# rampasek/DrVAE

Hardware: AMD Instinct MI355X
Metric: DrVAE ELBO training samples/sec (batch x L) (higher is better)
Workload: dtype f32; 1 GPU; cfg2: DrVAE bortezomib shape: 978 genes, z1=z3=100, enc-z1 800, dec-x 600, enc-z3/dec-z1 200, batch 150/GPU, L=2; global_batch=150, L=2, parallelism=dp1, launch=hipGraph replay, feed=resident, side_chain_cus=64, rccl_ranks=0, params=2321758

## Files before the change

### drvae_amd/csrc/gemm.hip

```cpp
#include "gemm_common.inc"

namespace {

#include "gemm_pipe.inc"


struct Operand {
    const float* base;
    int64_t ld;
    int n_line, n_pos;
};

__device__ __forceinline__ float4 ld_fast(const Operand& o, int line, int pos, int vec) {
    const float* p = o.base + (int64_t)line * o.ld + pos;
    if (vec == 4) return *reinterpret_cast<const float4*>(p);
    if (vec == 2) {
        const float2 a = *reinterpret_cast<const float2*>(p), b = *reinterpret_cast<const float2*>(p + 2);
        return make_float4(a.x, a.y, b.x, b.y);
    }
    return make_float4(p[0], p[1], p[2], p[3]);
}

__device__ __forceinline__ float4 ld_edge(const Operand& o, int line, int pos) {
    const bool lok = line < o.n_line;
    const float* row = o.base + (int64_t)(lok ? line : o.n_line - 1) * o.ld;
    float e[4];
#pragma unroll
    for (int j = 0; j < 4; ++j) {
        const int q = pos + j;
        const float v = row[q < o.n_pos ? q : o.n_pos - 1];
        e[j] = (lok && q < o.n_pos) ? v : 0.f;
    }
    return make_float4(e[0], e[1], e[2], e[3]);
}

template <int BM, int RPT>
__device__ __forceinline__ int heads_row0(int grp) { return (grp & 1) * (BM / 2) + (grp >> 1) * RPT; }

template <int BM, int BN, int KS, int NT>
__device__ __forceinline__ void heads_epilogue(const dv_gemm_desc& g, const dv_heads_epi& he, const float* red, int m0,
                                               int tn, int tiles_n, int pre_s0, int pre_s1) {
    constexpr int HB = BN / 2, RPT = BM / (NT / HB);
    constexpr bool PRE = (KS == 8 && BN == 32);
    static_assert(!PRE || RPT == 1, "prefetched bounds: one row per thread");
    static_assert((HB == 32 || HB == 16) && RPT >= 1, "half tile = 16 or 32 adjacent lanes");
    static_assert((NT / HB) % 2 == 0 && (BM / 2) % RPT == 0, "row groups come in pairs");
    const int tid = threadIdx.x, c = tid % HB, r0 = heads_row0<BM, RPT>(tid / HB);
    const int col0 = tn * HB + c, col1 = g.split + col0;
    const bool ok = col0 < g.split && col1 < g.N;
    const int cc0 = ok ? col0 : g.split - 1, cc1 = ok ? col1 : g.N - 1;
    float sc0 = 1.f, sc1 = 1.f, bi0 = 0.f, bi1 = 0.f;
    if (g.scale) {
        sc0 = g.scale[cc0];
        sc1 = g.scale[cc1];
    }
    if (g.bias) {
        bi0 = g.bias[cc0];
        bi1 = g.bias[cc1];
    }
    const bool use_res = g.resid != nullptr && col0 < g.resid_cols;
#pragma unroll
    for (int e = 0; e < RPT; ++e) {
        const int row = m0 + r0 + e;
        const bool rok = row < g.M;
        const int rc = rok ? row : g.M - 1;
        float v0 = 0.f, v1 = 0.f;
#pragma unroll
        for (int w = 0; w < KS; ++w) {
            v0 += red[(w * BM + r0 + e) * (BN + 1) + c];
            v1 += red[(w * BM + r0 + e) * (BN + 1) + HB + c];
        }
        float a0 = dv_act(g.act0, v0 * g.alpha * sc0 + bi0) + g.shift0;
        if (use_res) a0 += g.resid[(int64_t)rc * g.ldr + cc0];
        if (he.mode == DV_HEADS_NLL && g.act1 == DV_ACT_SOFTPLUS) {
            const float pre = v1 * g.alpha * sc1 + bi1;
            const float e_ = __expf(-fabsf(pre));
            const float r1 = __frcp_rn(1.f + e_);
            const float sd = fmaxf(pre, 0.f) + dv_log1p_hw(e_, r1) + g.shift1;
            const float sig = (pre >= 0.f ? 1.f : e_) * r1;
            const float is = __frcp_rn(sd);
            const float xv = he.x[(int64_t)(he.xidx ? he.xidx[rc] : rc) * he.ldx + cc0];
            const float cf = he.coef[rc];
            const float t = (xv - a0) * is;
            float acc = ok ? kLog2PiG + 2.f * __logf(sd) + t * t : 0.f;
            if (ok && rok) {
                g.C[(int64_t)row * g.ldc + col0] = cf * t * is;
                g.C[(int64_t)row * g.ldc + col1] = cf * (t * t - 1.f) * is * sig;
            }
#pragma unroll
            for (int off = HB / 2; off > 0; off >>= 1) acc += __shfl_xor(acc, off, 64);
            if (c == 0 && rok) he.part[(int64_t)row * tiles_n + tn] = -0.5f * acc;
            continue;
        }
        const float a1 = dv_act(g.act1, v1 * g.alpha * sc1 + bi1) + g.shift1;
        if (he.mode == DV_HEADS_SAMPLE) {
            if (ok && rok) {
                g.C[(int64_t)row * g.ldc + col0] = a0;
                g.C[(int64_t)row * g.ldc + col1] = a1;
                if (row < he.n_src) {
                    const float std_ = expf(0.5f * a1);
                    const int s0 = he.seg_ptr ? (PRE ? pre_s0 : he.seg_ptr[row]) : row;
                    const int s1 = he.seg_ptr ? (PRE ? pre_s1 : he.seg_ptr[row + 1]) : row + 1;
                    for (int t = s0; t < s1; ++t) {
                        const int64_t s = he.seg_rows ? he.seg_rows[t] : t;
                        const float z = he.eps[s * he.lde + col0] * std_ + a0;
                        he.out[s * he.ldo + col0] = z;
                        if (he.out2) he.out2[s * he.ldo2 + col0] = z - he.sub[s * he.lds + col0];
                        if (he.out3) {
                            const int t3 = he.out3_idx[s];
                            if (t3 >= 0) he.out3[(int64_t)t3 * he.ldo3 + col0] = z;
                        }
                        if (he.out4)
                            for (int u = he.out4_ptr[s]; u < he.out4_ptr[s + 1]; ++u) he.out4[(int64_t)u * he.ldo4 + col0] = z;
                    }
                }
            }
        } else {
            const float xv = he.x[(int64_t)(he.xidx ? he.xidx[rc] : rc) * he.ldx + cc0];
            const float cf = he.coef[rc];
            const float d = xv - a0, v = a1 * a1;
            float acc = ok ? kLog2PiG + logf(v) + d * d / v : 0.f;
            float gm = d / v, gs = -1.f / a1 + d * d / (v * a1);
            if (g.act1 != DV_ACT_IDENTITY) gs *= dv_dact_from_y(g.act1, a1 - g.shift1);
            gm *= cf;
            gs *= cf;
            if (ok && rok) {
                g.C[(int64_t)row * g.ldc + col0] = gm;
                g.C[(int64_t)row * g.ldc + col1] = gs;
            }
#pragma unroll
            for (int off = HB / 2; off > 0; off >>= 1) acc += __shfl_xor(acc, off, 64);
            if (c == 0 && rok) he.part[(int64_t)row * tiles_n + tn] = -0.5f * acc;
        }
    }
}

template <int BM, int BN, int BK, int KS, bool AKC, bool BKC, int PS = 0>
constexpr int gemm_smem_floats() {
    if constexpr (PS > 0) return PipeGeom<BM, BN, BK, BM / 32, BN / 32, KS, PS, AKC, BKC>::SMEM_FL;
    constexpr int stage = (AKC ? BM : BK) * ((AKC ? BK : BM) + 4) + (BKC ? BN : BK) * ((BKC ? BK : BN) + 4);
    constexpr int red = (KS > 1) ? KS * BM * (BN + 1) : 0;
    return 2 * stage > red ? 2 * stage : red;
}

template <int BM, int BN, int BK, int WM, int WN, int KS, bool AKC, bool BKC, bool PAIR = false, bool MI16 = false, int PS = 0>
__device__ __forceinline__ void gemm_body(const dv_gemm_desc& g, const LoadCfg& lc, float* smem, int bid, int nwg,
                                          const dv_heads_epi* he = nullptr) {
    static_assert(!PAIR || (AKC && BKC && KS > 1 && WM == 1 && WN == 1), "paired heads: forward layout, K-split tiling");
    constexpr int HB = BN / 2;
    static_assert(!MI16 || (KS == 1 && !PAIR), "16x16x4 tiles: unsplit K only");
    constexpr int TS = MI16 ? 16 : 32;
    constexpr int AR = MI16 ? 4 : 16;
// ... 82 lines not shown
        for (int p = 0; p < B_NP; ++p) {
            const int l = b_l + p * B_LPP;
            rb[p] = ld_edge(ob, BKC ? (PAIR ? bline(l) : n0 + l) : (k0 + l), BKC ? (k0 + b_c * 4) : (n0 + b_c * 4));
        }
    };
    auto stage_store = [&](float* buf, const float4 (&ra)[A_NP], const float4 (&rb)[B_NP]) {
        float* sA = buf;
        float* sB = buf + A_ELEMS;
#pragma unroll
        for (int p = 0; p < A_NP; ++p) {
            *reinterpret_cast<float4*>(&sA[(a_l + p * A_LPP) * LDA_S + a_c * 4]) = ra[p];
        }
#pragma unroll
        for (int p = 0; p < B_NP; ++p) {
            float4 v = rb[p];
            if (BM < 128 && !AKC && !BKC) {
                v.x = oc == 0 ? 1.f : v.x;
                v.y = oc == 1 ? 1.f : v.y;
                v.z = oc == 2 ? 1.f : v.z;
                v.w = oc == 3 ? 1.f : v.w;
            }
            *reinterpret_cast<float4*>(&sB[(b_l + p * B_LPP) * LDB_S + b_c * 4]) = v;
        }
    };

    typename std::conditional<MI16, f32x4, f32x16>::type acc[TM][TN];
#pragma unroll
    for (int i = 0; i < TM; ++i)
#pragma unroll
        for (int j = 0; j < TN; ++j)
#pragma unroll
            for (int r = 0; r < AR; ++r) acc[i][j][r] = 0.f;

    int pre_s0 = 0, pre_s1 = 0;
    if constexpr (PAIR && KS == 8 && BN == 32) {
        if (he->mode == DV_HEADS_SAMPLE && he->seg_ptr != nullptr) {
            const int prow = m0 + heads_row0<BM, 1>(tid / (BN / 2));
            if (prow < he->n_src && prow < g.M) {
                pre_s0 = he->seg_ptr[prow];
                pre_s1 = he->seg_ptr[prow + 1];
            }
        }
    }
    const int kb = ks_id * KW + lh * KH;
    auto read_frags = [&](const float* sA, float (&fa)[TM][KH], float (&fb)[TN][KH]) {
        const float* sB = sA + A_ELEMS;
#pragma unroll
        for (int i = 0; i < TM; ++i) {
            const int row = wm * TM * TS + i * TS + li;
#pragma unroll
            for (int s = 0; s < KH; s += 4) {
                if (AKC) {
                    const float4 v = *reinterpret_cast<const float4*>(&sA[row * LDA_S + kb + s]);
                    fa[i][s] = v.x;
                    fa[i][s + 1] = v.y;
                    fa[i][s + 2] = v.z;
                    fa[i][s + 3] = v.w;
                } else {
#pragma unroll
                    for (int e = 0; e < 4; ++e) fa[i][s + e] = sA[(kb + s + e) * LDA_S + row];
                }
            }
        }
#pragma unroll
        for (int j = 0; j < TN; ++j) {
            const int col = wn * TN * TS + j * TS + li;
#pragma unroll
            for (int s = 0; s < KH; s += 4) {
                if (BKC) {
                    const float4 v = *reinterpret_cast<const float4*>(&sB[col * LDB_S + kb + s]);
                    fb[j][s] = v.x;
                    fb[j][s + 1] = v.y;
                    fb[j][s + 2] = v.z;
                    fb[j][s + 3] = v.w;
                } else {
#pragma unroll
                    for (int e = 0; e < 4; ++e) fb[j][s + e] = sB[(kb + s + e) * LDB_S + col];
                }
            }
        }
    };
    auto mma = [&](const float (&fa)[TM][KH], const float (&fb)[TN][KH]) {
#pragma unroll
        for (int s = 0; s < KH; ++s)
#pragma unroll
            for (int i = 0; i < TM; ++i)
#pragma unroll
                for (int j = 0; j < TN; ++j) {
                    if constexpr (MI16)
                        acc[i][j] = __builtin_amdgcn_mfma_f32_16x16x4f32(fa[i][s], fb[j][s], acc[i][j], 0, 0, 0);
                    else if (DV_DBG & 2)
                        acc[i][j][s & 15] += fa[i][s] * fb[j][s];
                    else
                        acc[i][j] = __builtin_amdgcn_mfma_f32_32x32x2f32(fa[i][s], fb[j][s], acc[i][j], 0, 0, 0);
                }
    };
    auto compute = [&](const float* sA) {
        float fa[TM][KH], fb[TN][KH];
        read_frags(sA, fa, fb);
        mma(fa, fb);
    };

    const int nkt = (g.K + BK - 1) / BK, nfull = g.K / BK;
    float* const buf0 = smem;
    float* const buf1 = smem + STAGE;
    if constexpr (PS > 0) {
        if (!(DV_DBG & 64))
            pipe_loop<BM, BN, BK, WM, WN, KS, PS, AKC, BKC, (BM < 128 && !AKC && !BKC)>(
                g, smem, m0, n0, [&](int l) { return m0 + l < g.M ? m0 + l : g.M - 1; }, bline, acc);
        if (DV_DBG & 128) {
            if (acc[0][0][0] == 12345.678f) g.C[0] = acc[0][0][1];
            return;
        }
        __syncthreads();
    } else if (wg_fast && nfull >= 1) {
        const float* pa[A_NP];
        const float* pb[B_NP];
#pragma unroll
        for (int p = 0; p < A_NP; ++p) {
            const int l = a_l + p * A_LPP;
            int line = AKC ? (m0 + l) : l;
            if (AKC) line = line < g.M ? line : g.M - 1;
            pa[p] = g.A + (int64_t)line * g.lda + (AKC ? a_c * 4 : (m0 + a_c * 4 < g.M ? m0 + a_c * 4 : 0));
        }
#pragma unroll
        for (int p = 0; p < B_NP; ++p) {
            const int l = b_l + p * B_LPP;
            const int line = BKC ? bline(l) : l;
            pb[p] = g.B + (int64_t)line * g.ldb + (BKC ? b_c * 4 : (n0 + b_c * 4 < g.N ? n0 + b_c * 4 : 0));
        }
        const int64_t step_a = AKC ? (int64_t)BK : (int64_t)BK * g.lda;
        const int64_t step_b = BKC ? (int64_t)BK : (int64_t)BK * g.ldb;
        const int va = lc.vecA, vb = lc.vecB;
        auto ldv = [](const float* p, int vec) -> float4 {
            if (vec == 4) return *reinterpret_cast<const float4*>(p);
            if (vec == 2) {
                const float2 a = *reinterpret_cast<const float2*>(p), b = *reinterpret_cast<const float2*>(p + 2);
                return make_float4(a.x, a.y, b.x, b.y);
            }
            return make_float4(p[0], p[1], p[2], p[3]);
        };
        auto ldv_tail = [](const float* p, int vec, int left) -> float4 {
// ... 119 lines not shown
    if constexpr (MI16) {
#pragma unroll
        for (int i = 0; i < TM; ++i)
#pragma unroll
            for (int j = 0; j < TN; ++j) {
                float a4[4];
#pragma unroll
                for (int r = 0; r < 4; ++r) a4[r] = acc[i][j][r];
                const int rbase = m0 + wm * TM * TS + i * TS + 4 * lh;
                epi_store_col<4, (BM < 128)>(g, a4, n0 + wn * TN * TS + j * TS + li, [rbase](int r) { return rbase + r; });
            }
    } else if constexpr (KS == 1) {
#pragma unroll
        for (int i = 0; i < TM; ++i)
#pragma unroll
            for (int j = 0; j < TN; ++j) {
                float a16[16];
#pragma unroll
                for (int r = 0; r < 16; ++r) a16[r] = acc[i][j][r];
                const int rbase = m0 + wm * TM * 32 + i * 32 + 4 * lh;
                epi_store_col<16, (BM < 128)>(g, a16, n0 + wn * TN * 32 + j * 32 + li,
                                  [rbase](int r) { return rbase + (r & 3) + 8 * (r >> 2); });
            }
    } else {
        float* red = smem;
        if constexpr (PAIR) {
#pragma unroll
            for (int j = 0; j < TN; ++j)
#pragma unroll
                for (int r = 0; r < 16; ++r) {
                    const int row = (r & 3) + 8 * (r >> 2) + 4 * lh;
                    red[(ks_id * BM + row) * (BN + 1) + j * 32 + li] = acc[0][j][r];
                }
            __syncthreads();
            heads_epilogue<BM, BN, KS, NT>(g, *he, red, m0, tn, tiles_n, pre_s0, pre_s1);
            return;
        }
#pragma unroll
        for (int i = 0; i < TM; ++i)
#pragma unroll
            for (int j = 0; j < TN; ++j)
#pragma unroll
                for (int r = 0; r < 16; ++r) {
                    const int row = wm * TM * 32 + i * 32 + (r & 3) + 8 * (r >> 2) + 4 * lh;
                    const int col = wn * TN * 32 + j * 32 + li;
                    red[(ks_id * BM + row) * (BN + 1) + col] = acc[i][j][r];
                }
        __syncthreads();
        constexpr int RPT = BM / (NT / BN);
        const int col = tid % BN, r0 = (tid / BN) * RPT;
        float a4[RPT];
#pragma unroll
        for (int e = 0; e < RPT; ++e) {
            float v = 0.f;
#pragma unroll
            for (int w = 0; w < KS; ++w) v += red[(w * BM + r0 + e) * (BN + 1) + col];
            a4[e] = v;
        }
        const int rbase = m0 + r0;
        epi_store_col<RPT>(g, a4, n0 + col, [rbase](int r) { return rbase + r; });
    }
}


template <int BM, int BN, int BK, int WM, int WN, int KS, bool AKC, bool BKC, bool MI16 = false>
__global__ __launch_bounds__(64 * WM * WN * KS, (WM * WN * KS == 16) ? 4 : (BM >= 128 || BK >= 128) ? 2 : (BM * BN >= 6144) ? (WM * WN * KS) / 4 : (WM * WN * KS == 8 ? (BM * BN == 1024 ? DV_LB8 : 2) : (BK == 32 && BM == 32 ? ((AKC || BKC) ? DV_DENSE_WG : DV_DENSE_WG - 1) : 4))) void gemm_kernel(const dv_gemm_desc g, const LoadCfg lc) {
    __shared__ __attribute__((aligned(16))) float smem[gemm_smem_floats<BM, BN, BK, KS, AKC, BKC>()];
    publish_on_entry(g);
#if DV_STAGGER
    {
        const int ph = (blockIdx.x / DV_STAGGER) & 3;
        if (ph == 1) __builtin_amdgcn_s_sleep(6);
        if (ph == 2) __builtin_amdgcn_s_sleep(12);
        if (ph == 3) __builtin_amdgcn_s_sleep(18);
    }
#endif
    gemm_body<BM, BN, BK, WM, WN, KS, AKC, BKC, false, MI16>(g, lc, smem, blockIdx.x, gridDim.x);
}

#ifdef DV_LAB
template <int KS, int NBUF = 3>
__global__ __launch_bounds__(64 * KS, NBUF > 4 ? KS / 4 : (KS == 8 ? 2 : 4)) void gemm_dma_kernel(const dv_gemm_desc g, const LoadCfg lc) {
    constexpr int BM = 32, BN = 32, BK = 64, NT = 64 * KS, KW = BK / KS, KH = KW / 2;
    constexpr int TILE = 32 * BK, STAGE = 2 * TILE, RED = KS * BM * (BN + 1);
    constexpr int PIECES = 16 / KS;
    static_assert((NBUF - 2) * PIECES <= 63, "vmcnt is a 6-bit counter");
    __shared__ __attribute__((aligned(16))) float smem[NBUF * STAGE > RED ? NBUF * STAGE : RED];
    publish_on_entry(g);
    const int tiles_m = (g.M + BM - 1) / BM, tiles_n = (g.N + BN - 1) / BN;
    int tm, tn;
    tile_of_block(blockIdx.x, gridDim.x, tiles_m, tiles_n, lc.map, tm, tn);
    const int m0 = tm * BM, n0 = tn * BN;
    const int tid = threadIdx.x, lane = tid & 63, wave = tid >> 6;
// ... 171 lines not shown
    epi_store_col<RPT>(g, a4, n0 + col, [rbase](int r) { return rbase + r; });
}

#endif

template <int BM, int BN, int BK, int KS>
__global__ __launch_bounds__(64 * KS, KS == 8 ? 2 : (BK == 32 ? DV_DENSE_WG : 4)) void gemm_heads_kernel(const dv_gemm_desc g, const LoadCfg lc,
                                                               const dv_heads_epi he) {
    __shared__ __attribute__((aligned(16))) float smem[gemm_smem_floats<BM, BN, BK, KS, true, true>()];
    publish_on_entry(g);
    gemm_body<BM, BN, BK, 1, 1, KS, true, true, true>(g, lc, smem, blockIdx.x, gridDim.x, &he);
}

template <int BM, int BN, int BK, int WM, int WN, int KS, bool A1, bool B1, bool A2, bool B2>
__global__ __launch_bounds__(256, BK == 32 ? DV_DENSE_WG : 4) void gemm_pair_kernel(const dv_gemm_desc g1, const LoadCfg lc1, const dv_gemm_desc g2,
                                                        const LoadCfg lc2, int tiles1) {
    constexpr int S1 = gemm_smem_floats<BM, BN, BK, KS, A1, B1>(), S2 = gemm_smem_floats<BM, BN, BK, KS, A2, B2>();
    __shared__ __attribute__((aligned(16))) float smem[S1 > S2 ? S1 : S2];
    publish_on_entry(g1);
    if ((int)blockIdx.x < tiles1)
        gemm_body<BM, BN, BK, WM, WN, KS, A1, B1>(g1, lc1, smem, blockIdx.x, tiles1);
    else
        gemm_body<BM, BN, BK, WM, WN, KS, A2, B2>(g2, lc2, smem, blockIdx.x - tiles1, gridDim.x - tiles1);
}

template <int BM, int BN, int BK, int KS, bool AKC, bool BKC, int PS, int WPS>
__global__ __launch_bounds__(64 * KS * (BM / 32) * (BN / 32), WPS) void gemm_kpipe_kernel(const dv_gemm_desc g, const LoadCfg lc) {
    __shared__ __attribute__((aligned(1024))) float smem[gemm_smem_floats<BM, BN, BK, KS, AKC, BKC, PS>()];
    publish_on_entry(g);
    gemm_body<BM, BN, BK, BM / 32, BN / 32, KS, AKC, BKC, false, false, PS>(g, lc, smem, blockIdx.x, gridDim.x);
}

template <int BM, int BN, int BK, int KS, int PS, int WPS>
__global__ __launch_bounds__(64 * KS, WPS) void gemm_heads_pipe_kernel(const dv_gemm_desc g, const LoadCfg lc, const dv_heads_epi he) {
    __shared__ __attribute__((aligned(1024))) float smem[gemm_smem_floats<BM, BN, BK, KS, true, true, PS>()];
    publish_on_entry(g);
    gemm_body<BM, BN, BK, 1, 1, KS, true, true, true, false, PS>(g, lc, smem, blockIdx.x, gridDim.x, &he);
}

template <int BM, int BN, int BK, int KS, bool A1, bool B1, bool A2, bool B2, int PS, int WPS>
__global__ __launch_bounds__(256, WPS) void gemm_pair_pipe_kernel(const dv_gemm_desc g1, const LoadCfg lc1, const dv_gemm_desc g2,
                                                                    const LoadCfg lc2, int tiles1) {
    constexpr int S1 = gemm_smem_floats<BM, BN, BK, KS, A1, B1, PS>(), S2 = gemm_smem_floats<BM, BN, BK, KS, A2, B2, PS>();
    __shared__ __attribute__((aligned(1024))) float smem[S1 > S2 ? S1 : S2];
    publish_on_entry(g1);
    if ((int)blockIdx.x < tiles1)
        gemm_body<BM, BN, BK, 1, 1, KS, A1, B1, false, false, PS>(g1, lc1, smem, blockIdx.x, tiles1);
    else
        gemm_body<BM, BN, BK, 1, 1, KS, A2, B2, false, false, PS>(g2, lc2, smem, blockIdx.x - tiles1, gridDim.x - tiles1);
}

inline int vec_width(const void* p, int64_t ld) {
    const uintptr_t a = reinterpret_cast<uintptr_t>(p);
    if ((a & 15) == 0 && (ld & 3) == 0) return 4;
    if ((a & 7) == 0 && (ld & 1) == 0) return 2;
    return 1;
}

const dv_gemm_tune k_default_tune = {0, {-1, 0, 0, 0, 0, 0, 0, 0, 0, 0}};
inline const dv_gemm_tune& tune_of(const dv_gemm_desc& g) { return g.tune != nullptr ? *g.tune : k_default_tune; }
inline int lds_pad(const dv_gemm_desc& g, int bm, int tiles) { return (bm <= 32 && tiles >= 512) ? tune_of(g).opt[1] : 0; }

inline int cols_eff(const dv_gemm_desc& g) { return g.N + ((g.flags & DV_FLAG_ONES_COL) ? DV_ONES_OFF(g) + 1 : 0); }

template <int BM, int BN, int BK, int WM, int WN, int KS, bool MI16 = false>
int launch_cfg(const dv_gemm_desc& g, const LoadCfg& lc, hipStream_t st) {
    const int tiles = ((g.M + BM - 1) / BM) * ((cols_eff(g) + BN - 1) / BN);
// ... 366 lines not shown
```

### drvae_amd/csrc/gemm_common.inc

```
#pragma once
#include <type_traits>

#include "dv_common.h"

typedef float f32x16 __attribute__((ext_vector_type(16)));
typedef float f32x4 __attribute__((ext_vector_type(4)));

#ifndef DV_DBG
#define DV_DBG 0
#endif
#ifndef DV_STAGGER
#define DV_STAGGER 0
#endif
#ifndef DV_STAMP
#define DV_STAMP 0
#endif
#ifndef DV_LB8
#define DV_LB8 2
#endif
#ifndef DV_DENSE_WG
#define DV_DENSE_WG 7
#endif
#if DV_STAMP
__device__ unsigned long long* dv_stamp_buf = nullptr;
// ... 28 lines not shown
    int stagger = 0;
};

__device__ __forceinline__ void tile_of_block(int bid, int nwg, int tiles_m, int tiles_n, int map, int& tm,
                                              int& tn) {
    int t = bid;
    if (map == 1 && nwg >= 16) {
        const int x = bid & 7, j = bid >> 3, base = nwg >> 3, rem = nwg & 7;
        t = x * base + (x < rem ? x : rem) + j;
        if (tiles_n >= tiles_m) {
            const int cw = (tiles_n + 7) >> 3, per = cw * tiles_m, c = t / per, r = t - c * per;
            const int w = (tiles_n - c * cw) < cw ? (tiles_n - c * cw) : cw;
            tm = r / w;
            tn = c * cw + r % w;
        } else {
            const int ch = (tiles_m + 7) >> 3, per = ch * tiles_n, c = t / per, r = t - c * per;
            const int h = (tiles_m - c * ch) < ch ? (tiles_m - c * ch) : ch;
            tn = r / h;
            tm = c * ch + r % h;
        }
        return;
    }
    if (map >= 2) {
        const int gm = map, per = gm * tiles_n, grp = t / per, first = grp * gm;
        const int h = (tiles_m - first) < gm ? (tiles_m - first) : gm, r = t - grp * per;
        tm = first + r % h;
        tn = r / h;
        return;
    }
    tm = t / tiles_n;
    tn = t % tiles_n;
}

template <int NR, bool ONES = true, typename RowOf>
__device__ __forceinline__ void epi_store_col(const dv_gemm_desc& g, const float (&acc)[NR], int col, RowOf row_of) {
    const bool cok = col < g.N;
    const int cc = cok ? col : g.N - 1;
    if (ONES && (g.flags & DV_FLAG_ONES_COL) && col == g.N + DV_ONES_OFF(g)) {
#pragma unroll
        for (int r = 0; r < NR; ++r) {
            const int row = row_of(r);
            if (row < g.M)
                g.a_colsum[row] = (g.colsum_beta != 0.f ? g.colsum_beta * g.a_colsum[row] : 0.f) + acc[r];
        }
        return;
    }
    if (g.epilogue == DV_EPI_KLQ) {
        if (!cok || col >= g.split) return;
#pragma unroll
        for (int r = 0; r < NR; ++r) {
            const int row = row_of(r);
            if (row < g.M) {
                const float rv = g.scale[row];
                const float c = g.bias[row] * (rv > g.shift0 ? 1.f : (rv == g.shift0 ? 0.5f : 0.f));
                const float mq = g.yref[(int64_t)row * g.ldy + col], lq = g.yref[(int64_t)row * g.ldy + g.split + col];
                const float v = acc[r] * g.alpha;
                float tq_mu = c * (mq * 1.f), tq_sd = c * (-0.5f * (1.f - expf(lq) * 1.f));
                tq_mu += v;
                tq_sd += v * g.resid[(int64_t)row * g.ldr + col] * (0.5f * expf(0.5f * lq));
                g.C[(int64_t)row * g.ldc + col] = tq_mu;
                g.C[(int64_t)row * g.ldc + g.split + col] = tq_sd;
            }
        }
        return;
    }
    const bool first = col < g.split;
    const int act = first ? g.act0 : g.act1;
    const float shift = first ? g.shift0 : g.shift1;
    float sc = 1.f, bi = 0.f;
    if (g.epilogue == DV_EPI_FWD) {
        if (g.scale) sc = g.scale[cc];
        if (g.bias) bi = g.bias[cc];
    }
    float ex[NR], old[NR];
    const float* exsrc = nullptr;
    int64_t exld = 0;
    if (g.epilogue == DV_EPI_FWD && g.resid) {
        exsrc = g.resid;
        exld = g.ldr;
    } else if (g.epilogue == DV_EPI_BWD) {
        exsrc = g.yref;
        exld = g.ldy;
    }
    const bool use_ex = exsrc != nullptr;
    const bool use_old = g.beta != 0.f;
    const int exc = (g.epilogue == DV_EPI_FWD && use_ex) ? (col < g.resid_cols ? col : 0) : cc;
#pragma unroll
    for (int r = 0; r < NR; ++r) {
        const int row = row_of(r), rc = row < g.M ? row : g.M - 1;
        ex[r] = use_ex ? exsrc[(int64_t)rc * exld + exc] : 0.f;
        old[r] = use_old ? g.C[(int64_t)rc * g.ldc + cc] : 0.f;
    }
#pragma unroll
    for (int r = 0; r < NR; ++r) {
        const int row = row_of(r);
        float v = acc[r] * g.alpha;
        if (g.epilogue == DV_EPI_FWD) {
            v = dv_act(act, v * sc + bi) + shift;
            if (use_ex && col < g.resid_cols) v += ex[r];
        } else if (g.epilogue == DV_EPI_BWD) {
            v *= dv_dact_from_y(act, ex[r] - shift);
        }
        if (use_old) v += g.beta * old[r];
        if (cok && row < g.M) g.C[(int64_t)row * g.ldc + col] = v;
    }
}

__device__ __forceinline__ void publish_on_entry(const dv_gemm_desc& g) {
    if (g.pub_flag != nullptr && blockIdx.x == 0 && threadIdx.x == 0)
        __hip_atomic_store(g.pub_flag, g.pub_ctr[0] + g.pub_add, __ATOMIC_RELEASE, __HIP_MEMORY_SCOPE_AGENT);
}

}
```

### drvae_amd/csrc/gemm_pipe.inc

```

template <int BM, int BN, int BK, int WM, int WN, int KS, int S, bool AKC, bool BKC>
struct PipeGeom {
    static constexpr int NW = WM * WN * KS, NT = 64 * NW;
    static constexpr int TM = BM / WM / 32, TN = BN / WN / 32;
    static constexpr int KW = BK / KS, KH = KW / 2, G = KH / 4;
    static constexpr int A_FL = BM * BK, B_FL = BN * BK, STAGE_FL = A_FL + B_FL;
    static constexpr int PA = A_FL / 256, PB = B_FL / 256, P = (PA + PB) / NW;
    static constexpr int CPR = BK / 4;
    static constexpr int RED_FL = (KS > 1) ? KS * BM * (BN + 1) : 0;
    static constexpr int SMEM_FL = S * STAGE_FL > RED_FL ? S * STAGE_FL : RED_FL;
    static_assert(KH % 4 == 0 && G >= 1, "a lane half holds whole 16-B chunks of k");
    static_assert((PA + PB) % NW == 0 && P >= 1, "pieces divide over the waves");
    static_assert(CPR == 4 || CPR == 8 || CPR == 16, "BK = 16, 32 or 64");
    static_assert(TM == 1 || TM == 2 || TM == 4, "row-contiguous reads are 4, 8 or 16 B");
    static_assert(TN == 1 || TN == 2 || TN == 4, "row-contiguous reads are 4, 8 or 16 B");
    static_assert(AKC || (256 % BM == 0 && BM <= 256), "row-contiguous A: whole k lines per piece");
    static_assert(BKC || (256 % BN == 0 && BN <= 256), "row-contiguous B: whole k lines per piece");
    static_assert((S - 2) * P <= 63 && S >= 2, "vmcnt is a 6-bit counter");
};

template <int CPR>
__device__ __forceinline__ int pipe_sw(int row) {
    return (row / (16 / CPR)) & (CPR - 1);
}

template <int N>
__device__ __forceinline__ void pipe_wait_vm() {
    asm volatile("s_waitcnt vmcnt(%0)" ::"n"(N) : "memory");
}

template <int BM, int BN, int BK, int WM, int WN, int KS, int S, bool AKC, bool BKC, bool ONES = false, typename LineA,
          typename LineB>
__device__ __forceinline__ void pipe_loop(const dv_gemm_desc& g, float* smem, int m0, int n0, LineA a_line,
                                          LineB b_line, f32x16 (&acc)[BM / WM / 32][BN / WN / 32]) {
    using PG = PipeGeom<BM, BN, BK, WM, WN, KS, S, AKC, BKC>;
    constexpr int TM = PG::TM, TN = PG::TN, G = PG::G, P = PG::P, CPR = PG::CPR, NW = PG::NW;
    const int tid = threadIdx.x, lane = tid & 63;
    const int wave = __builtin_amdgcn_readfirstlane(tid >> 6);
    const int li = lane & 31, lh = lane >> 5;
    const int ks_id = wave / (WM * WN), wm = (wave % (WM * WN)) / WN, wn = wave % WN;

    unsigned voff[P];
    int kofs[P];
    bool live[P];
    const bool ones_on = ONES && (g.flags & DV_FLAG_ONES_COL) != 0;
    const int n_ones = g.N + DV_ONES_OFF(g);
#pragma unroll
    for (int i = 0; i < P; ++i) {
        const int q = wave + i * NW;
        const bool isA = q < PG::PA;
        const int pq = isA ? q : q - PG::PA;
        const bool kc = isA ? AKC : BKC;
        const int64_t ld = isA ? g.lda : g.ldb;
        live[i] = true;
        if (kc) {
            const int row_t = pq * (64 / CPR) + lane / CPR;
            const int c = (lane % CPR) ^ pipe_sw<CPR>(row_t);
            const int T = isA ? TM : TN, wq = row_t / (T * 32), jq = (row_t / 32) % T, lq = row_t % 32;
            const int line = isA ? a_line(wq * T * 32 + T * lq + jq) : b_line(wq * T * 32 + T * lq + jq);
            kofs[i] = c * 4;
            voff[i] = (unsigned)(((int64_t)line * ld + c * 4) * 4);
        } else {
            const int R = isA ? BM : BN;
            const int line_t = pq * (256 / R) + lane / (R / 4), rc = lane % (R / 4);
            const int r0 = isA ? m0 : n0, lim = isA ? g.M : g.N;
            const int col = r0 + rc * 4 < lim ? r0 + rc * 4 : 0;
            kofs[i] = line_t;
// ... 69 lines not shown
                }
            }
        }
    };
    auto read_group = [&](const float* stage, int gi, float (&fa)[TM][4], float (&fb)[TN][4]) {
        read_ops(stage, gi, fa, fb, 0, NR);
    };
    auto mma = [&](const float (&fa)[TM][4], const float (&fb)[TN][4], int lo, int hi) {
#pragma unroll
        for (int s = 0; s < 4; ++s)
#pragma unroll
            for (int i = 0; i < TM; ++i)
#pragma unroll
                for (int j = 0; j < TN; ++j) {
                    const int n = (s * TM + i) * TN + j;
                    if (n >= lo && n < hi) {
                        if (DV_DBG & 32) {
                            acc[i][j][0] += fa[i][s] + fb[j][s];
                        } else {
                            acc[i][j] = __builtin_amdgcn_mfma_f32_32x32x2f32(fa[i][s], fb[j][s], acc[i][j], 0, 0, 0);
                        }
                    }
                }
    };
    constexpr int NM = 4 * TM * TN;
    constexpr int RPM = (NR + NM - 1) / NM > 2 ? (NR + NM - 1) / NM : 2, NSL = (NR + RPM - 1) / RPM;
    static_assert(NSL <= NM, "reads dealt out over the group's MFMAs");
    const int nkt = (g.K + BK - 1) / BK;
    if constexpr (ONES) {
        if (ones_on && n0 <= n_ones && n_ones < n0 + BN && tid < S * BK)
            *reinterpret_cast<float4*>(&smem[(tid / BK) * PG::STAGE_FL + PG::A_FL + (tid % BK) * BN + (n_ones - n0)]) =
                make_float4(1.f, 1.f, 1.f, 1.f);
    }
#pragma unroll
    for (int t = 0; t < S; ++t) {
        if (k_issued + BK <= g.K) {
#pragma unroll
            for (int i = 0; i < P; ++i) issue_piece(std::true_type{}, i, t * PG::STAGE_FL * 4);
        } else {
#pragma unroll
            for (int i = 0; i < P; ++i) issue_piece(std::false_type{}, i, t * PG::STAGE_FL * 4);
        }
        issued();
    }
    asm volatile("s_waitcnt lgkmcnt(0)" ::: "memory");
    pipe_wait_vm<(S - 1) * P>();
    __builtin_amdgcn_s_barrier();
    float fa0[TM][4], fb0[TN][4], fa1[TM][4], fb1[TN][4];
    read_group(smem, 0, fa0, fb0);
    int sc = 0;
    auto tile = [&](auto full, float (&xa)[TM][4], float (&xb)[TN][4], float (&ya)[TM][4], float (&yb)[TN][4]) {
        const float* cur = smem + sc * PG::STAGE_FL;
        const int sn = sc + 1 == S ? 0 : sc + 1;
        const float* nxt = smem + sn * PG::STAGE_FL;
#pragma unroll
        for (int gi = 0; gi < G; ++gi) {
            float(&ca)[TM][4] = (gi & 1) ? ya : xa;
            float(&cb)[TN][4] = (gi & 1) ? yb : xb;
            float(&na)[TM][4] = (gi & 1) ? xa : ya;
            float(&nb)[TN][4] = (gi & 1) ? xb : yb;
            if (gi + 1 < G) {
                mma(ca, cb, 0, 1);
                __builtin_amdgcn_sched_barrier(0);
#pragma unroll
                for (int q = 0; q < NSL; ++q) {
                    read_ops(cur, gi + 1, na, nb, q * RPM, (q + 1) * RPM);
                    __builtin_amdgcn_sched_barrier(0);
                    if (q + 1 < NSL) {
                        mma(ca, cb, 1 + q, 2 + q);
                        __builtin_amdgcn_sched_barrier(0);
                    }
                }
                mma(ca, cb, NSL, NM);
                __builtin_amdgcn_sched_barrier(0);
            } else {
                asm volatile("s_waitcnt lgkmcnt(0)" ::: "memory");
                pipe_wait_vm<(S - 2) * P>();
                __builtin_amdgcn_s_barrier();
                asm volatile("" ::: "memory");
                mma(ca, cb, 0, 1);
                __builtin_amdgcn_sched_barrier(0);
#pragma unroll
                for (int q = 0; q < NSL; ++q) {
                    read_ops(nxt, 0, na, nb, q * RPM, (q + 1) * RPM);
                    __builtin_amdgcn_sched_barrier(0);
                    if (q + 1 < NSL) {
                        mma(ca, cb, 1 + q, 2 + q);
                        __builtin_amdgcn_sched_barrier(0);
                    }
                }
                const unsigned sb = sc * PG::STAGE_FL * 4;
                constexpr int M0 = NSL, ML = NM - M0;
#pragma unroll
                for (int i = 0; i < P; ++i) {
                    mma(ca, cb, M0 + i * ML / (P + 1), M0 + (i + 1) * ML / (P + 1));
                    __builtin_amdgcn_sched_barrier(0);
                    issue_piece(full, i, sb);
                    __builtin_amdgcn_sched_barrier(0);
                }
                mma(ca, cb, M0 + P * ML / (P + 1), NM);
                __builtin_amdgcn_sched_barrier(0);
                issued();
            }
        }
        sc = sn;
    };
    const int nfast = g.K / BK - S;
    int kt = 0;
    if constexpr (G % 2 == 0) {
        for (; kt < nfast; ++kt) tile(std::true_type{}, fa0, fb0, fa1, fb1);
        for (; kt < nkt; ++kt) tile(std::false_type{}, fa0, fb0, fa1, fb1);
    } else {
        for (; kt + 1 < nfast; kt += 2) {
            tile(std::true_type{}, fa0, fb0, fa1, fb1);
            tile(std::true_type{}, fa1, fb1, fa0, fb0);
        }
        for (; kt + 1 < nkt; kt += 2) {
            tile(std::false_type{}, fa0, fb0, fa1, fb1);
            tile(std::false_type{}, fa1, fb1, fa0, fb0);
        }
        if (kt < nkt) tile(std::false_type{}, fa0, fb0, fa1, fb1);
    }
    pipe_wait_vm<0>();
}

template <int BM, int BN, int WM, int WN, bool AKC, bool BKC>
__device__ __forceinline__ void pipe_epilogue(const dv_gemm_desc& g, int m0, int n0,
                                              const f32x16 (&acc)[BM / WM / 32][BN / WN / 32]) {
    constexpr int TM = BM / WM / 32, TN = BN / WN / 32;
    const int lane = threadIdx.x & 63, wave = threadIdx.x >> 6, li = lane & 31, lh = lane >> 5;
    const int wm = (wave % (WM * WN)) / WN, wn = wave % WN;
    const int rw = m0 + wm * TM * 32, cw = n0 + wn * TN * 32;
    const bool vec_ok = TN > 1 && g.epilogue == DV_EPI_PLAIN && g.beta == 0.f && (g.N % TN) == 0 &&
                        (g.ldc % TN) == 0 && (reinterpret_cast<uintptr_t>(g.C) % (4 * TN)) == 0;
    if (vec_ok) {
        if (cw + TN * li >= g.N) return;
#pragma unroll
        for (int i = 0; i < TM; ++i)
#pragma unroll
            for (int r = 0; r < 16; ++r) {
                const int rho = (r & 3) + 8 * (r >> 2) + 4 * lh;
                const int row = rw + TM * rho + i;
                if (row < g.M) {
                    float* p = g.C + (int64_t)row * g.ldc + cw + TN * li;
                    if constexpr (TN == 4) {
                        *reinterpret_cast<float4*>(p) = make_float4(acc[i][0][r] * g.alpha, acc[i][1][r] * g.alpha,
                                                                    acc[i][2][r] * g.alpha, acc[i][3][r] * g.alpha);
                    } else {
                        *reinterpret_cast<float2*>(p) = make_float2(acc[i][0][r] * g.alpha, acc[i][TN - 1][r] * g.alpha);
                    }
                }
            }
        return;
    }
// ... 154 lines not shown
```

Before: 1.636 million samples/s.

## Prefetch epilogue operands during GEMM main loop and trim pipeline tail

Adds staged early loads of epilogue operands (scale, bias, residual, x, coef, segment rows, eps and sub values for the heads kernel, and generic column operands for split-K pipe kernels). These loads are issued inside the pipelined K loop so their latency overlaps the MMAs instead of stalling the epilogue. The two-slot pipeline also gets dedicated tail modes that skip useless prefetch issues and waits on the last tiles, and the heads kernel's launch-bounds occupancy argument now scales with KS. In exchange, register pressure rises, which could cut occupancy or cause spills.

```diff
diff --git a/drvae_amd/csrc/gemm.hip b/drvae_amd/csrc/gemm.hip
--- a/drvae_amd/csrc/gemm.hip
+++ b/drvae_amd/csrc/gemm.hip
@@ -37,9 +37,70 @@
 template <int BM, int RPT>
 __device__ __forceinline__ int heads_row0(int grp) { return (grp & 1) * (BM / 2) + (grp >> 1) * RPT; }
 
+constexpr int kHeadsPreRows = 4;
+struct HeadsPre {
+    float sc0, sc1, bi0, bi1, res, xv, cf;
+    int xrow, s0, s1;
+    int srow[kHeadsPreRows], t3[kHeadsPreRows], u0[kHeadsPreRows], u1[kHeadsPreRows];
+    float eps[kHeadsPreRows], sub[kHeadsPreRows];
+};
+
+template <int BM, int BN>
+__device__ __forceinline__ void heads_early(const dv_gemm_desc& g, const dv_heads_epi& he, int m0, int tn, int stage,
+                                            HeadsPre& hp) {
+    constexpr int HB = BN / 2;
+    const int tid = threadIdx.x, c = tid % HB, row = m0 + heads_row0<BM, 1>(tid / HB);
+    const int col0 = tn * HB + c, col1 = g.split + col0;
+    const bool ok = col0 < g.split && col1 < g.N, rok = row < g.M;
+    const int cc0 = ok ? col0 : g.split - 1, cc1 = ok ? col1 : g.N - 1, rc = rok ? row : g.M - 1;
+    if (stage == 0) {
+        hp.sc0 = hp.sc1 = 1.f;
+        hp.bi0 = hp.bi1 = hp.res = 0.f;
+        if (g.scale) {
+            hp.sc0 = g.scale[cc0];
+            hp.sc1 = g.scale[cc1];
+        }
+        if (g.bias) {
+            hp.bi0 = g.bias[cc0];
+            hp.bi1 = g.bias[cc1];
+        }
+        if (g.resid != nullptr) hp.res = g.resid[(int64_t)rc * g.ldr + (col0 < g.resid_cols ? cc0 : 0)];
+        hp.s0 = hp.s1 = 0;
+        if (he.mode == DV_HEADS_NLL) {
+            hp.xrow = he.xidx ? he.xidx[rc] : rc;
+            hp.cf = he.coef[rc];
+        } else {
+            const bool on = ok && rok && row < he.n_src;
+            hp.s0 = he.seg_ptr ? ld_or_zero(on, he.seg_ptr + row) : (on ? row : 0);
+            hp.s1 = he.seg_ptr ? ld_or_zero(on, he.seg_ptr + row + 1) : (on ? row + 1 : 0);
+        }
+    } else if (stage == 1) {
+        if (he.mode == DV_HEADS_NLL) {
+            hp.xv = he.x[(int64_t)hp.xrow * he.ldx + cc0];
+        } else {
+#pragma unroll
+            for (int j = 0; j < kHeadsPreRows; ++j)
+                hp.srow[j] = he.seg_rows ? ld_or_zero(hp.s0 + j < hp.s1, he.seg_rows + hp.s0 + j) : hp.s0 + j;
+        }
+    } else if (he.mode == DV_HEADS_SAMPLE) {
+#pragma unroll
+        for (int j = 0; j < kHeadsPreRows; ++j) {
+            const bool on = hp.s0 + j < hp.s1;
+            const int64_t s = hp.srow[j];
+            hp.eps[j] = ld_or_zero(on, he.eps + s * he.lde + col0);
+            if (he.out2) hp.sub[j] = ld_or_zero(on, he.sub + s * he.lds + col0);
+            if (he.out3) hp.t3[j] = ld_or_zero(on, he.out3_idx + s);
+            if (he.out4) {
+                hp.u0[j] = ld_or_zero(on, he.out4_ptr + s);
+                hp.u1[j] = ld_or_zero(on, he.out4_ptr + s + 1);
+            }
+        }
+    }
+}
+
 template <int BM, int BN, int KS, int NT>
 __device__ __forceinline__ void heads_epilogue(const dv_gemm_desc& g, const dv_heads_epi& he, const float* red, int m0,
-                                               int tn, int tiles_n, int pre_s0, int pre_s1) {
+                                               int tn, int tiles_n, const HeadsPre& hp) {
     constexpr int HB = BN / 2, RPT = BM / (NT / HB);
     constexpr bool PRE = (KS == 8 && BN == 32);
     static_assert(!PRE || RPT == 1, "prefetched bounds: one row per thread");
@@ -50,13 +111,20 @@
     const bool ok = col0 < g.split && col1 < g.N;
     const int cc0 = ok ? col0 : g.split - 1, cc1 = ok ? col1 : g.N - 1;
     float sc0 = 1.f, sc1 = 1.f, bi0 = 0.f, bi1 = 0.f;
-    if (g.scale) {
-        sc0 = g.scale[cc0];
-        sc1 = g.scale[cc1];
-    }
-    if (g.bias) {
-        bi0 = g.bias[cc0];
-        bi1 = g.bias[cc1];
+    if constexpr (PRE) {
+        sc0 = hp.sc0;
+        sc1 = hp.sc1;
+        bi0 = hp.bi0;
+        bi1 = hp.bi1;
+    } else {
+        if (g.scale) {
+            sc0 = g.scale[cc0];
+            sc1 = g.scale[cc1];
+        }
+        if (g.bias) {
+            bi0 = g.bias[cc0];
+            bi1 = g.bias[cc1];
+        }
     }
     const bool use_res = g.resid != nullptr && col0 < g.resid_cols;
 #pragma unroll
@@ -71,7 +139,7 @@
             v1 += red[(w * BM + r0 + e) * (BN + 1) + HB + c];
         }
         float a0 = dv_act(g.act0, v0 * g.alpha * sc0 + bi0) + g.shift0;
-        if (use_res) a0 += g.resid[(int64_t)rc * g.ldr + cc0];
+        if (use_res) a0 += PRE ? hp.res : g.resid[(int64_t)rc * g.ldr + cc0];
         if (he.mode == DV_HEADS_NLL && g.act1 == DV_ACT_SOFTPLUS) {
             const float pre = v1 * g.alpha * sc1 + bi1;
             const float e_ = __expf(-fabsf(pre));
@@ -79,8 +147,8 @@
             const float sd = fmaxf(pre, 0.f) + dv_log1p_hw(e_, r1) + g.shift1;
             const float sig = (pre >= 0.f ? 1.f : e_) * r1;
             const float is = __frcp_rn(sd);
-            const float xv = he.x[(int64_t)(he.xidx ? he.xidx[rc] : rc) * he.ldx + cc0];
-            const float cf = he.coef[rc];
+            const float xv = PRE ? hp.xv : he.x[(int64_t)(he.xidx ? he.xidx[rc] : rc) * he.ldx + cc0];
+            const float cf = PRE ? hp.cf : he.coef[rc];
             const float t = (xv - a0) * is;
             float acc = ok ? kLog2PiG + 2.f * __logf(sd) + t * t : 0.f;
             if (ok && rok) {
@@ -99,9 +167,25 @@
                 g.C[(int64_t)row * g.ldc + col1] = a1;
                 if (row < he.n_src) {
                     const float std_ = expf(0.5f * a1);
-                    const int s0 = he.seg_ptr ? (PRE ? pre_s0 : he.seg_ptr[row]) : row;
-                    const int s1 = he.seg_ptr ? (PRE ? pre_s1 : he.seg_ptr[row + 1]) : row + 1;
-                    for (int t = s0; t < s1; ++t) {
+                    const int s0 = PRE ? hp.s0 : (he.seg_ptr ? he.seg_ptr[row] : row);
+                    const int s1 = PRE ? hp.s1 : (he.seg_ptr ? he.seg_ptr[row + 1] : row + 1);
+                    if constexpr (PRE) {
+#pragma unroll
+                        for (int j = 0; j < kHeadsPreRows; ++j) {
+                            if (s0 + j >= s1) break;
+                            const int64_t s = hp.srow[j];
+                            const float z = hp.eps[j] * std_ + a0;
+                            he.out[s * he.ldo + col0] = z;
+                            if (he.out2) he.out2[s * he.ldo2 + col0] = z - hp.sub[j];
+                            if (he.out3) {
+                                const int t3 = hp.t3[j];
+                                if (t3 >= 0) he.out3[(int64_t)t3 * he.ldo3 + col0] = z;
+                            }
+                            if (he.out4)
+                                for (int u = hp.u0[j]; u < hp.u1[j]; ++u) he.out4[(int64_t)u * he.ldo4 + col0] = z;
+                        }
+                    }
+                    for (int t = PRE ? s0 + kHeadsPreRows : s0; t < s1; ++t) {
                         const int64_t s = he.seg_rows ? he.seg_rows[t] : t;
                         const float z = he.eps[s * he.lde + col0] * std_ + a0;
                         he.out[s * he.ldo + col0] = z;
@@ -116,8 +200,8 @@
                 }
             }
         } else {
-            const float xv = he.x[(int64_t)(he.xidx ? he.xidx[rc] : rc) * he.ldx + cc0];
-            const float cf = he.coef[rc];
+            const float xv = PRE ? hp.xv : he.x[(int64_t)(he.xidx ? he.xidx[rc] : rc) * he.ldx + cc0];
+            const float cf = PRE ? hp.cf : he.coef[rc];
             const float d = xv - a0, v = a1 * a1;
             float acc = ok ? kLog2PiG + logf(v) + d * d / v : 0.f;
             float gm = d / v, gs = -1.f / a1 + d * d / (v * a1);
@@ -266,15 +350,22 @@
 #pragma unroll
             for (int r = 0; r < AR; ++r) acc[i][j][r] = 0.f;
 
-    int pre_s0 = 0, pre_s1 = 0;
-    if constexpr (PAIR && KS == 8 && BN == 32) {
-        if (he->mode == DV_HEADS_SAMPLE && he->seg_ptr != nullptr) {
-            const int prow = m0 + heads_row0<BM, 1>(tid / (BN / 2));
-            if (prow < he->n_src && prow < g.M) {
-                pre_s0 = he->seg_ptr[prow];
-                pre_s1 = he->seg_ptr[prow + 1];
-            }
-        }
+    constexpr bool HPRE = PAIR && KS == 8 && BN == 32;
+    constexpr bool EPRE = !PAIR && PS == 2 && KS > 1 && BK == 64;
+    constexpr int RPT_E = KS > 1 ? BM / (NT / BN) : 1;
+    HeadsPre hp;
+    EpiOperands<RPT_E> eops;
+    auto early = [&](int stage) __attribute__((always_inline)) {
+        if constexpr (HPRE) {
+            heads_early<BM, BN>(g, *he, m0, tn, stage, hp);
+        } else if constexpr (EPRE) {
+            const int rbase = m0 + (tid / BN) * RPT_E;
+            if (stage == 0) epi_load_col<RPT_E>(g, n0 + tid % BN, [rbase](int r) { return rbase + r; }, eops);
+        }
+    };
+    if constexpr (HPRE && PS == 0) {
+        early(0);
+        early(1);
     }
     const int kb = ks_id * KW + lh * KH;
     auto read_frags = [&](const float* sA, float (&fa)[TM][KH], float (&fb)[TN][KH]) {
@@ -339,9 +430,14 @@
     float* const buf0 = smem;
     float* const buf1 = smem + STAGE;
     if constexpr (PS > 0) {
-        if (!(DV_DBG & 64))
-            pipe_loop<BM, BN, BK, WM, WN, KS, PS, AKC, BKC, (BM < 128 && !AKC && !BKC)>(
-                g, smem, m0, n0, [&](int l) { return m0 + l < g.M ? m0 + l : g.M - 1; }, bline, acc);
+        if (!(DV_DBG & 64)) {
+            auto aline = [&](int l) { return m0 + l < g.M ? m0 + l : g.M - 1; };
+            if constexpr (HPRE || EPRE)
+                pipe_loop<BM, BN, BK, WM, WN, KS, PS, AKC, BKC, (BM < 128 && !AKC && !BKC)>(g, smem, m0, n0, aline, bline, acc, early);
+            else
+                pipe_loop<BM, BN, BK, WM, WN, KS, PS, AKC, BKC, (BM < 128 && !AKC && !BKC)>(g, smem, m0, n0, aline, bline, acc);
+        }
+        if constexpr (HPRE) early(2);
         if (DV_DBG & 128) {
             if (acc[0][0][0] == 12345.678f) g.C[0] = acc[0][0][1];
             return;
@@ -527,8 +623,9 @@
                     const int row = (r & 3) + 8 * (r >> 2) + 4 * lh;
                     red[(ks_id * BM + row) * (BN + 1) + j * 32 + li] = acc[0][j][r];
                 }
+            if constexpr (HPRE && PS == 0) early(2);
             __syncthreads();
-            heads_epilogue<BM, BN, KS, NT>(g, *he, red, m0, tn, tiles_n, pre_s0, pre_s1);
+            heads_epilogue<BM, BN, KS, NT>(g, *he, red, m0, tn, tiles_n, hp);
             return;
         }
 #pragma unroll
@@ -553,7 +650,10 @@
             a4[e] = v;
         }
         const int rbase = m0 + r0;
-        epi_store_col<RPT>(g, a4, n0 + col, [rbase](int r) { return rbase + r; });
+        if constexpr (EPRE)
+            epi_store_col_pre<RPT>(g, a4, n0 + col, [rbase](int r) { return rbase + r; }, eops);
+        else
+            epi_store_col<RPT>(g, a4, n0 + col, [rbase](int r) { return rbase + r; });
     }
 }
 
@@ -791,7 +891,7 @@
 }
 
 template <int BM, int BN, int BK, int KS, int PS, int WPS>
-__global__ __launch_bounds__(64 * KS, WPS) void gemm_heads_pipe_kernel(const dv_gemm_desc g, const LoadCfg lc, const dv_heads_epi he) {
+__global__ __launch_bounds__(64 * KS, WPS * KS / 4) void gemm_heads_pipe_kernel(const dv_gemm_desc g, const LoadCfg lc, const dv_heads_epi he) {
     __shared__ __attribute__((aligned(1024))) float smem[gemm_smem_floats<BM, BN, BK, KS, true, true, PS>()];
     publish_on_entry(g);
     gemm_body<BM, BN, BK, 1, 1, KS, true, true, true, false, PS>(g, lc, smem, blockIdx.x, gridDim.x, &he);
diff --git a/drvae_amd/csrc/gemm_common.inc b/drvae_amd/csrc/gemm_common.inc
--- a/drvae_amd/csrc/gemm_common.inc
+++ b/drvae_amd/csrc/gemm_common.inc
@@ -84,6 +84,30 @@
     tn = t % tiles_n;
 }
 
+__device__ __forceinline__ void epi_klq_store(const dv_gemm_desc& g, int row, int col, float a, float rv, float bv, float mq,
+                                              float lq, float rs) {
+    const float c = bv * (rv > g.shift0 ? 1.f : (rv == g.shift0 ? 0.5f : 0.f));
+    const float v = a * g.alpha;
+    float tq_mu = c * (mq * 1.f), tq_sd = c * (-0.5f * (1.f - expf(lq) * 1.f));
+    tq_mu += v;
+    tq_sd += v * rs * (0.5f * expf(0.5f * lq));
+    g.C[(int64_t)row * g.ldc + col] = tq_mu;
+    g.C[(int64_t)row * g.ldc + g.split + col] = tq_sd;
+}
+
+__device__ __forceinline__ float epi_col_value(const dv_gemm_desc& g, int act, float shift, float sc, float bi, float a,
+                                               float ex, float old, bool add_ex, bool use_old) {
+    float v = a * g.alpha;
+    if (g.epilogue == DV_EPI_FWD) {
+        v = dv_act(act, v * sc + bi) + shift;
+        if (add_ex) v += ex;
+    } else if (g.epilogue == DV_EPI_BWD) {
+        v *= dv_dact_from_y(act, ex - shift);
+    }
+    if (use_old) v += g.beta * old;
+    return v;
+}
+
 template <int NR, bool ONES = true, typename RowOf>
 __device__ __forceinline__ void epi_store_col(const dv_gemm_desc& g, const float (&acc)[NR], int col, RowOf row_of) {
     const bool cok = col < g.N;
@@ -102,17 +126,9 @@
 #pragma unroll
         for (int r = 0; r < NR; ++r) {
             const int row = row_of(r);
-            if (row < g.M) {
-                const float rv = g.scale[row];
-                const float c = g.bias[row] * (rv > g.shift0 ? 1.f : (rv == g.shift0 ? 0.5f : 0.f));
-                const float mq = g.yref[(int64_t)row * g.ldy + col], lq = g.yref[(int64_t)row * g.ldy + g.split + col];
-                const float v = acc[r] * g.alpha;
-                float tq_mu = c * (mq * 1.f), tq_sd = c * (-0.5f * (1.f - expf(lq) * 1.f));
-                tq_mu += v;
-                tq_sd += v * g.resid[(int64_t)row * g.ldr + col] * (0.5f * expf(0.5f * lq));
-                g.C[(int64_t)row * g.ldc + col] = tq_mu;
-                g.C[(int64_t)row * g.ldc + g.split + col] = tq_sd;
-            }
+            if (row < g.M)
+                epi_klq_store(g, row, col, acc[r], g.scale[row], g.bias[row], g.yref[(int64_t)row * g.ldy + col],
+                              g.yref[(int64_t)row * g.ldy + g.split + col], g.resid[(int64_t)row * g.ldr + col]);
         }
         return;
     }
@@ -146,14 +162,87 @@
 #pragma unroll
     for (int r = 0; r < NR; ++r) {
         const int row = row_of(r);
-        float v = acc[r] * g.alpha;
-        if (g.epilogue == DV_EPI_FWD) {
-            v = dv_act(act, v * sc + bi) + shift;
-            if (use_ex && col < g.resid_cols) v += ex[r];
-        } else if (g.epilogue == DV_EPI_BWD) {
-            v *= dv_dact_from_y(act, ex[r] - shift);
-        }
-        if (use_old) v += g.beta * old[r];
+        const float v = epi_col_value(g, act, shift, sc, bi, acc[r], ex[r], old[r], use_ex && col < g.resid_cols, use_old);
+        if (cok && row < g.M) g.C[(int64_t)row * g.ldc + col] = v;
+    }
+}
+
+template <int NR>
+struct EpiOperands {
+    float sc, bi;
+    float ex[NR], old[NR];
+    float rv[NR], bv[NR], lq[NR], rs[NR];
+};
+
+template <typename T>
+__device__ __forceinline__ T ld_or_zero(bool valid, const T* p) {
+    static_assert(sizeof(T) == 4, "one word of the zero chunk");
+    return *(valid ? p : reinterpret_cast<const T*>(dv_zero_chunk));
+}
+
+template <int NR, typename RowOf>
+__device__ __forceinline__ void epi_load_col(const dv_gemm_desc& g, int col, RowOf row_of, EpiOperands<NR>& o) {
+    const bool cok = col < g.N;
+    const int cc = cok ? col : g.N - 1;
+    const bool klq = g.epilogue == DV_EPI_KLQ, fwd = g.epilogue == DV_EPI_FWD, bwd = g.epilogue == DV_EPI_BWD;
+    const float sc = ld_or_zero(fwd && g.scale != nullptr, g.scale + cc);
+    o.sc = (fwd && g.scale != nullptr) ? sc : 1.f;
+    o.bi = ld_or_zero(fwd && g.bias != nullptr, g.bias + cc);
+    const float* exsrc = fwd ? g.resid : g.yref;
+    const int64_t exld = fwd ? g.ldr : g.ldy;
+    const bool use_ex = (fwd || bwd || klq) && exsrc != nullptr, use_old = g.beta != 0.f && !klq;
+    const int ck = (cok && col < g.split) ? col : 0;
+    const int exc = klq ? ck : (fwd ? (col < g.resid_cols ? col : 0) : cc);
+#pragma unroll
+    for (int r = 0; r < NR; ++r) {
+        const int row = row_of(r), rc = row < g.M ? row : g.M - 1;
+        o.ex[r] = ld_or_zero(use_ex, exsrc + (int64_t)rc * exld + exc);
+        o.old[r] = ld_or_zero(use_old, g.C + (int64_t)rc * g.ldc + cc);
+        o.rv[r] = o.bv[r] = o.lq[r] = o.rs[r] = 0.f;
+    }
+    if (klq) {
+#pragma unroll
+        for (int r = 0; r < NR; ++r) {
+            const int row = row_of(r), rc = row < g.M ? row : g.M - 1;
+            o.rv[r] = g.scale[rc];
+            o.bv[r] = g.bias[rc];
+            o.lq[r] = g.yref[(int64_t)rc * g.ldy + g.split + ck];
+            o.rs[r] = g.resid[(int64_t)rc * g.ldr + ck];
+        }
+    }
+}
+
+template <int NR, bool ONES = true, typename RowOf>
+__device__ __forceinline__ void epi_store_col_pre(const dv_gemm_desc& g, const float (&acc)[NR], int col, RowOf row_of,
+                                                  const EpiOperands<NR>& o) {
+    const bool cok = col < g.N;
+    if (ONES && (g.flags & DV_FLAG_ONES_COL) && col == g.N + DV_ONES_OFF(g)) {
+#pragma unroll
+        for (int r = 0; r < NR; ++r) {
+            const int row = row_of(r);
+            if (row < g.M)
+                g.a_colsum[row] = (g.colsum_beta != 0.f ? g.colsum_beta * g.a_colsum[row] : 0.f) + acc[r];
+        }
+        return;
+    }
+    if (g.epilogue == DV_EPI_KLQ) {
+        if (!cok || col >= g.split) return;
+#pragma unroll
+        for (int r = 0; r < NR; ++r) {
+            const int row = row_of(r);
+            if (row < g.M) epi_klq_store(g, row, col, acc[r], o.rv[r], o.bv[r], o.ex[r], o.lq[r], o.rs[r]);
+        }
+        return;
+    }
+    const bool first = col < g.split;
+    const int act = first ? g.act0 : g.act1;
+    const float shift = first ? g.shift0 : g.shift1;
+    const bool use_ex = g.epilogue == DV_EPI_BWD || (g.epilogue == DV_EPI_FWD && g.resid != nullptr);
+    const bool use_old = g.beta != 0.f;
+#pragma unroll
+    for (int r = 0; r < NR; ++r) {
+        const int row = row_of(r);
+        const float v = epi_col_value(g, act, shift, o.sc, o.bi, acc[r], o.ex[r], o.old[r], use_ex && col < g.resid_cols, use_old);
         if (cok && row < g.M) g.C[(int64_t)row * g.ldc + col] = v;
     }
 }
diff --git a/drvae_amd/csrc/gemm_pipe.inc b/drvae_amd/csrc/gemm_pipe.inc
--- a/drvae_amd/csrc/gemm_pipe.inc
+++ b/drvae_amd/csrc/gemm_pipe.inc
@@ -29,10 +29,14 @@
     asm volatile("s_waitcnt vmcnt(%0)" ::"n"(N) : "memory");
 }
 
+struct pipe_no_early {
+    __device__ __forceinline__ void operator()(int) const {}
+};
+
 template <int BM, int BN, int BK, int WM, int WN, int KS, int S, bool AKC, bool BKC, bool ONES = false, typename LineA,
-          typename LineB>
+          typename LineB, typename Early = pipe_no_early>
 __device__ __forceinline__ void pipe_loop(const dv_gemm_desc& g, float* smem, int m0, int n0, LineA a_line,
-                                          LineB b_line, f32x16 (&acc)[BM / WM / 32][BN / WN / 32]) {
+                                          LineB b_line, f32x16 (&acc)[BM / WM / 32][BN / WN / 32], Early early = Early{}) {
     using PG = PipeGeom<BM, BN, BK, WM, WN, KS, S, AKC, BKC>;
     constexpr int TM = PG::TM, TN = PG::TN, G = PG::G, P = PG::P, CPR = PG::CPR, NW = PG::NW;
     const int tid = threadIdx.x, lane = tid & 63;
@@ -168,8 +172,10 @@
             *reinterpret_cast<float4*>(&smem[(tid / BK) * PG::STAGE_FL + PG::A_FL + (tid % BK) * BN + (n_ones - n0)]) =
                 make_float4(1.f, 1.f, 1.f, 1.f);
     }
+    early(0);
 #pragma unroll
     for (int t = 0; t < S; ++t) {
+        if (S == 2 && k_issued >= g.K) break;
         if (k_issued + BK <= g.K) {
 #pragma unroll
             for (int i = 0; i < P; ++i) issue_piece(std::true_type{}, i, t * PG::STAGE_FL * 4);
@@ -180,12 +186,18 @@
         issued();
     }
     asm volatile("s_waitcnt lgkmcnt(0)" ::: "memory");
-    pipe_wait_vm<(S - 1) * P>();
+    if (S == 2 && nkt < 2)
+        pipe_wait_vm<0>();
+    else
+        pipe_wait_vm<(S - 1) * P>();
     __builtin_amdgcn_s_barrier();
+    early(1);
     float fa0[TM][4], fb0[TN][4], fa1[TM][4], fb1[TN][4];
     read_group(smem, 0, fa0, fb0);
     int sc = 0;
-    auto tile = [&](auto full, float (&xa)[TM][4], float (&xb)[TN][4], float (&ya)[TM][4], float (&yb)[TN][4]) {
+    auto tile = [&](auto mode, float (&xa)[TM][4], float (&xb)[TN][4], float (&ya)[TM][4], float (&yb)[TN][4]) __attribute__((always_inline)) {
+        constexpr int MODE = decltype(mode)::value;
+        static_assert(MODE <= 1 || S == 2, "only the two-slot ring ends at K");
         const float* cur = smem + sc * PG::STAGE_FL;
         const int sn = sc + 1 == S ? 0 : sc + 1;
         const float* nxt = smem + sn * PG::STAGE_FL;
@@ -209,6 +221,9 @@
                 }
                 mma(ca, cb, NSL, NM);
                 __builtin_amdgcn_sched_barrier(0);
+            } else if constexpr (MODE == 3) {
+                mma(ca, cb, 0, NM);
+                __builtin_amdgcn_sched_barrier(0);
             } else {
                 asm volatile("s_waitcnt lgkmcnt(0)" ::: "memory");
                 pipe_wait_vm<(S - 2) * P>();
@@ -227,35 +242,63 @@
                 }
                 const unsigned sb = sc * PG::STAGE_FL * 4;
                 constexpr int M0 = NSL, ML = NM - M0;
-#pragma unroll
-                for (int i = 0; i < P; ++i) {
-                    mma(ca, cb, M0 + i * ML / (P + 1), M0 + (i + 1) * ML / (P + 1));
+                if constexpr (MODE == 2) {
+                    mma(ca, cb, M0, NM);
                     __builtin_amdgcn_sched_barrier(0);
-                    issue_piece(full, i, sb);
+                } else {
+#pragma unroll
+                    for (int i = 0; i < P; ++i) {
+                        mma(ca, cb, M0 + i * ML / (P + 1), M0 + (i + 1) * ML / (P + 1));
+                        __builtin_amdgcn_sched_barrier(0);
+                        issue_piece(std::integral_constant<bool, MODE == 0>{}, i, sb);
+                        __builtin_amdgcn_sched_barrier(0);
+                    }
+                    mma(ca, cb, M0 + P * ML / (P + 1), NM);
                     __builtin_amdgcn_sched_barrier(0);
-                }
-                mma(ca, cb, M0 + P * ML / (P + 1), NM);
-                __builtin_amdgcn_sched_barrier(0);
-                issued();
+                    issued();
+                }
             }
         }
         sc = sn;
     };
     const int nfast = g.K / BK - S;
+    using TileFull = std::integral_constant<int, 0>;
+    using TileRagged = std::integral_constant<int, 1>;
     int kt = 0;
-    if constexpr (G % 2 == 0) {
-        for (; kt < nfast; ++kt) tile(std::true_type{}, fa0, fb0, fa1, fb1);
-        for (; kt < nkt; ++kt) tile(std::false_type{}, fa0, fb0, fa1, fb1);
+    if constexpr (S == 2) {
+        auto tail = [&](int k, float (&xa)[TM][4], float (&xb)[TN][4], float (&ya)[TM][4], float (&yb)[TN][4]) __attribute__((always_inline)) {
+            if (k < nfast) tile(TileFull{}, xa, xb, ya, yb);
+            else if (k + 2 < nkt) tile(TileRagged{}, xa, xb, ya, yb);
+            else if (k + 1 < nkt) tile(std::integral_constant<int, 2>{}, xa, xb, ya, yb);
+            else tile(std::integral_constant<int, 3>{}, xa, xb, ya, yb);
+        };
+        if constexpr (G % 2 == 0) {
+            for (; kt < nfast; ++kt) tile(TileFull{}, fa0, fb0, fa1, fb1);
+            for (; kt < nkt; ++kt) tail(kt, fa0, fb0, fa1, fb1);
+        } else {
+            for (; kt + 1 < nfast; kt += 2) {
+                tile(TileFull{}, fa0, fb0, fa1, fb1);
+                tile(TileFull{}, fa1, fb1, fa0, fb0);
+            }
+            for (; kt < nkt; kt += 2) {
+                tail(kt, fa0, fb0, fa1, fb1);
+                if (kt + 1 < nkt) tail(kt + 1, fa1, fb1, fa0, fb0);
+            }
+        }
+        return;
+    } else if constexpr (G % 2 == 0) {
+        for (; kt < nfast; ++kt) tile(TileFull{}, fa0, fb0, fa1, fb1);
+        for (; kt < nkt; ++kt) tile(TileRagged{}, fa0, fb0, fa1, fb1);
     } else {
         for (; kt + 1 < nfast; kt += 2) {
-            tile(std::true_type{}, fa0, fb0, fa1, fb1);
-            tile(std::true_type{}, fa1, fb1, fa0, fb0);
+            tile(TileFull{}, fa0, fb0, fa1, fb1);
+            tile(TileFull{}, fa1, fb1, fa0, fb0);
         }
         for (; kt + 1 < nkt; kt += 2) {
-            tile(std::false_type{}, fa0, fb0, fa1, fb1);
-            tile(std::false_type{}, fa1, fb1, fa0, fb0);
-        }
-        if (kt < nkt) tile(std::false_type{}, fa0, fb0, fa1, fb1);
+            tile(TileRagged{}, fa0, fb0, fa1, fb1);
+            tile(TileRagged{}, fa1, fb1, fa0, fb0);
+        }
+        if (kt < nkt) tile(TileRagged{}, fa0, fb0, fa1, fb1);
     }
     pipe_wait_vm<0>();
 }
```

Result: no change. 1.643 million samples/s (median of 6 runs) (+0.4%).
